# calderpg/voxelized_geometry_tools

Hardware: AMD Instinct MI355X
Metric: Mvoxels/s for 1024^3 float SDF extract @1 GPU; % HBM roofline (higher is better)
Workload: dtype int32; 1 GPU; 1024^3 float SDF, D1 spheres seed 42, res 0.01, device-resident; workload_key=c4, parallelism=single GPU, edt_variant=0

## Files before the change

### voxelized_geometry_tools_amd/csrc/edt_sweep_kernels.hip

```cpp
#include "edt_device.hpp"
#include "edt_line_geom.hpp"

#include <cstdlib>
#include <type_traits>

namespace vgt
{
namespace
{
#ifndef VGT_SWEEP_BAND
#define VGT_SWEEP_BAND 16
#endif
#ifndef VGT_SWEEP_RING
#define VGT_SWEEP_RING 32
#endif
#ifndef VGT_SWEEP_CHUNK
#define VGT_SWEEP_CHUNK 8
#endif
#ifndef VGT_SWEEP_WAVES
#define VGT_SWEEP_WAVES 4
#endif
#ifndef VGT_SWEEP_GROUP
#define VGT_SWEEP_GROUP 2
#endif
constexpr int kBand = VGT_SWEEP_BAND;
constexpr int kWord = 32;
#ifndef VGT_SWEEP_RING_WIDE
#define VGT_SWEEP_RING_WIDE 16
#endif
#ifndef VGT_SWEEP_CHUNK_WIDE
#define VGT_SWEEP_CHUNK_WIDE 4
#endif
#ifndef VGT_SWEEP_GROUPS
#define VGT_SWEEP_GROUPS 8
#endif
constexpr int kSweepGroups = VGT_SWEEP_GROUPS;
constexpr int kCounterStride = 32;
constexpr int kMaxSweepSlots = 4096;
template <bool kPacked>
struct RingShape
{
  static constexpr int kRing = kPacked ? VGT_SWEEP_RING : VGT_SWEEP_RING_WIDE;
  static constexpr int kChunk = kPacked ? VGT_SWEEP_CHUNK : VGT_SWEEP_CHUNK_WIDE;
  static_assert(kBand % kChunk == 0 && kRing >= 4 * kChunk && (kRing & (kRing - 1)) == 0 && kChunk % 4 == 0, "sizes");
};
constexpr int kFar = 32768;
static_assert(kWord % kBand == 0 && kBand % 2 == 0, "sizes");
#ifdef VGT_HOST_EMULATION
uint64_t class_band_tally[3] = {0, 0, 0};
#endif


template <bool kPacked>
struct Codec;
template <>
struct Codec<true>
{
  using Entry = uint32_t;
  static constexpr int32_t kSentinelG = (1 << 22) - 3;
  static __device__ __forceinline__ Entry Pack(int32_t G, int row)
  {
    return (static_cast<uint32_t>(G) << 10) | static_cast<uint32_t>(row);
  }
  static __device__ __forceinline__ int32_t G(Entry e) { return static_cast<int32_t>(e >> 10); }
  static __device__ __forceinline__ int Row(Entry e) { return static_cast<int>(e & 1023u); }
  static __device__ __forceinline__ Entry Unknown() { return ~0u; }
  static __device__ __forceinline__ bool IsUnknown(Entry e) { return e == ~0u; }
};
template <>
struct Codec<false>
{
  using Entry = uint2;
  static constexpr int32_t kSentinelG = 1 << 30;
  static __device__ __forceinline__ Entry Pack(int32_t G, int row)
  {
    return make_uint2(static_cast<uint32_t>(G), static_cast<uint32_t>(row));
  }
  static __device__ __forceinline__ int32_t G(Entry e) { return static_cast<int32_t>(e.x); }
  static __device__ __forceinline__ int Row(Entry e) { return static_cast<int>(e.y); }
  static __device__ __forceinline__ Entry Unknown() { return make_uint2(0u, ~0u); }
  static __device__ __forceinline__ bool IsUnknown(Entry e) { return e.y == ~0u; }
};

#ifndef VGT_SWEEP_NT
#define VGT_SWEEP_NT 3
#endif
__device__ __forceinline__ void StoreQuad(uint4* p, uint32_t a, uint32_t b, uint32_t c, uint32_t d)
{
#if defined(VGT_HOST_EMULATION) || !(VGT_SWEEP_NT & 8)
  *p = make_uint4(a, b, c, d);
#else
  using Raw = uint32_t __attribute__((ext_vector_type(4)));
  Raw r;
  r.x = a; r.y = b; r.z = c; r.w = d;
  __builtin_nontemporal_store(r, reinterpret_cast<Raw*>(p));
#endif
}
__device__ __forceinline__ uint4 LoadQuad(const uint4* p)
{
#if defined(VGT_HOST_EMULATION) || !(VGT_SWEEP_NT & 8)
  return *p;
#else
  using Raw = uint32_t __attribute__((ext_vector_type(4)));
  const Raw r = __builtin_nontemporal_load(reinterpret_cast<const Raw*>(p));
  return make_uint4(r.x, r.y, r.z, r.w);
#endif
}
__device__ __forceinline__ void StorePair(uint2* p, uint32_t a, uint32_t b)
{
#if defined(VGT_HOST_EMULATION) || !(VGT_SWEEP_NT & 4)
  *p = make_uint2(a, b);
#else
  using Raw = uint32_t __attribute__((ext_vector_type(2)));
  Raw r;
  r.x = a; r.y = b;
  __builtin_nontemporal_store(r, reinterpret_cast<Raw*>(p));
#endif
}
__device__ __forceinline__ uint2 LoadPair(const uint2* p)
{
#if defined(VGT_HOST_EMULATION) || !(VGT_SWEEP_NT & 4)
  return *p;
#else
  using Raw = uint32_t __attribute__((ext_vector_type(2)));
  const Raw r = __builtin_nontemporal_load(reinterpret_cast<const Raw*>(p));
  return make_uint2(r.x, r.y);
#endif
}

template <int N>
__device__ __forceinline__ void StoreChunk(uint32_t* dst, const uint32_t (&e)[N])
{
#pragma unroll
  for (int j = 0; j < N / 4; j++)
    StoreQuad(reinterpret_cast<uint4*>(dst) + j, e[4 * j], e[4 * j + 1], e[4 * j + 2], e[4 * j + 3]);
}
template <int N>
__device__ __forceinline__ void LoadChunk(const uint32_t* src, uint32_t (&e)[N])
{
#pragma unroll
  for (int j = 0; j < N / 4; j++)
  {
    const uint4 a = LoadQuad(reinterpret_cast<const uint4*>(src) + j);
    e[4 * j] = a.x;
    e[4 * j + 1] = a.y;
    e[4 * j + 2] = a.z;
    e[4 * j + 3] = a.w;
  }
}
template <int N>
__device__ __forceinline__ void StoreChunk(uint2* dst, const uint2 (&e)[N])
{
#pragma unroll
  for (int j = 0; j < N / 2; j++)
    StoreQuad(reinterpret_cast<uint4*>(dst) + j, e[2 * j].x, e[2 * j].y, e[2 * j + 1].x, e[2 * j + 1].y);
}
template <int N>
__device__ __forceinline__ void LoadChunk(const uint2* src, uint2 (&e)[N])
{
#pragma unroll
  for (int j = 0; j < N / 2; j++)
  {
    const uint4 a = LoadQuad(reinterpret_cast<const uint4*>(src) + j);
    e[2 * j] = make_uint2(a.x, a.y);
    e[2 * j + 1] = make_uint2(a.z, a.w);
  }
}

#ifdef VGT_HOST_EMULATION
#define VGT_GLOBAL
#else
#define VGT_GLOBAL __attribute__((address_space(1)))
#endif
template <typename T>
__device__ __forceinline__ VGT_GLOBAL T* UniformPointer(const VGT_GLOBAL T* p)
{
  const uint64_t v = reinterpret_cast<uint64_t>(p);
  const uint32_t lo = __builtin_amdgcn_readfirstlane(static_cast<uint32_t>(v));
  const uint32_t hi = __builtin_amdgcn_readfirstlane(static_cast<uint32_t>(v >> 32));
  return reinterpret_cast<VGT_GLOBAL T*>((static_cast<uint64_t>(hi) << 32) | lo);
}
template <typename T>
__device__ __forceinline__ VGT_GLOBAL T* GlobalPointer(T* p)
{
#ifdef VGT_HOST_EMULATION
  return p;
#else
  return reinterpret_cast<VGT_GLOBAL T*>(reinterpret_cast<uint64_t>(p));
#endif
}

__device__ __forceinline__ int32_t Mad24Uniform(int32_t a, int32_t b_uniform, int32_t c)
{
#ifdef VGT_HOST_EMULATION
  return a * b_uniform + c;
#else
  int32_t d;
  asm("v_mad_i32_i24 %0, %1, %2, %3" : "=v"(d) : "v"(a), "s"(b_uniform), "v"(c));
  return d;
#endif
}

__device__ __forceinline__ int32_t FreshCopy(int32_t v)
{
#ifdef VGT_HOST_EMULATION
  return v;
#else
  int32_t d;
  asm("v_mov_b32 %0, %1" : "=v"(d) : "v"(v));
  return d;
#endif
}

template <bool kInPlace>
__device__ __forceinline__ uint32_t PinnedOffset(uint32_t& byte_offset)
{
#ifndef VGT_HOST_EMULATION
  if constexpr (kInPlace)
    asm volatile("" : "+v"(byte_offset));
  else
  {
    uint32_t copy = byte_offset;
    asm volatile("" : "+v"(copy));
    return copy;
  }
#endif
  return byte_offset;
}
template <typename T>
__device__ __forceinline__ const VGT_GLOBAL T* LaneAddress(const VGT_GLOBAL T* row, uint32_t& byte_offset)
{
  return reinterpret_cast<const VGT_GLOBAL T*>(reinterpret_cast<const VGT_GLOBAL unsigned char*>(row) +
                                                PinnedOffset<false>(byte_offset));
}
template <typename T>
__device__ __forceinline__ VGT_GLOBAL T* LaneAddress(VGT_GLOBAL T* row, uint32_t& byte_offset)
{
  return reinterpret_cast<VGT_GLOBAL T*>(reinterpret_cast<VGT_GLOBAL unsigned char*>(row) +
                                         PinnedOffset<true>(byte_offset));
}

__device__ __forceinline__ uint32_t AbsDiffPlusOne(uint32_t a, uint32_t b_uniform)
{
  return (max(a, b_uniform) - min(a, b_uniform)) + 1u;
}
__device__ __forceinline__ uint32_t SpreadLaneMask(uint64_t mask_uniform, [[maybe_unused]] int lane)
{
#ifdef VGT_HOST_EMULATION
  return ((mask_uniform >> lane) & 1ull) ? ~0u : 0u;
#else
  return __builtin_amdgcn_inverse_ballot_w64(mask_uniform) ? ~0u : 0u;
#endif
}

__device__ __forceinline__ uint32_t LowBits(int bits)
{
  return (bits >= 32) ? ~0u : ((1u << bits) - 1u);
}

#if defined(VGT_HOST_EMULATION) || !(VGT_SWEEP_NT & 1)
#define VGT_STREAM_LOAD(p) (*(p))
#else
#define VGT_STREAM_LOAD(p) __builtin_nontemporal_load(p)
#endif
#if defined(VGT_HOST_EMULATION) || !(VGT_SWEEP_NT & 2)
#define VGT_STREAM_STORE(v, p) (*(p) = (v))
#else
#define VGT_STREAM_STORE(v, p) __builtin_nontemporal_store(v, p)
#endif

#ifdef VGT_HOST_EMULATION
#define VGT_COLD_PATH()
#define VGT_MIN_F32(acc, v) acc = fminf(acc, v)
#define VGT_MAX_F32(acc, v) acc = fmaxf(acc, v)
#define VGT_MIN3_F32(acc, a, b) acc = fminf(acc, fminf(a, b))
#define VGT_MAX3_F32(acc, a, b) acc = fmaxf(acc, fmaxf(a, b))
#else
#define VGT_COLD_PATH() asm volatile("; rare path")
#define VGT_MIN_F32(acc, v) asm("v_min_f32 %0, %0, %1" : "+v"(acc) : "v"(v))
#define VGT_MAX_F32(acc, v) asm("v_max_f32 %0, %0, %1" : "+v"(acc) : "v"(v))
#define VGT_MIN3_F32(acc, a, b) asm("v_min3_f32 %0, %0, %1, %2" : "+v"(acc) : "v"(a), "v"(b))
#define VGT_MAX3_F32(acc, a, b) asm("v_max3_f32 %0, %0, %1, %2" : "+v"(acc) : "v"(a), "v"(b))
#endif


__device__ __forceinline__ void WaveMinMax(float lo_value, float hi_value, uint32_t* minmax_enc)
{
  uint32_t lo = 0xffffffffu, hi = 0u;
  if (lo_value <= hi_value)
  {
    lo = EncodeOrdered(lo_value);
    hi = EncodeOrdered(hi_value);
  }
#ifdef VGT_HOST_EMULATION
  minmax_enc[0] = min(minmax_enc[0], lo);
  minmax_enc[1] = max(minmax_enc[1], hi);
#else
  for (int off = kWaveSize / 2; off > 0; off >>= 1)
  {
    lo = min(lo, static_cast<uint32_t>(__shfl_xor(static_cast<int>(lo), off)));
    hi = max(hi, static_cast<uint32_t>(__shfl_xor(static_cast<int>(hi), off)));
  }
  if (threadIdx.x == 0)
  {
    atomicMin(&minmax_enc[0], lo);
    atomicMax(&minmax_enc[1], hi);
  }
#endif
}

template <typename InT, typename OutT, bool kFinal, bool kPacked, bool kPlain>
__global__ __launch_bounds__(kWaveSize, VGT_SWEEP_WAVES) void SweepPassKernel(const InT* __restrict__ in,
                                                                            OutT* __restrict__ out,
                                                                            unsigned char* __restrict__ spill,
                                                                            uint2* __restrict__ word_info,
                                                                            uint32_t* __restrict__ minmax_enc,
                                                                            int* __restrict__ work_counter,
                                                                            const SweepGeom g)
{
  using C = Codec<kPacked>;
  using Entry = typename C::Entry;
  constexpr bool kRecords = std::is_same<InT, ClassRecord>::value;
  static_assert(!(kRecords && kFinal), "records feed the Y pass");
  constexpr int kRing = RingShape<kPacked>::kRing;
  constexpr int kChunk = RingShape<kPacked>::kChunk;
  constexpr int32_t kLimit = C::kSentinelG;
  constexpr int kEntryBytes = static_cast<int>(sizeof(Entry));
  constexpr int kShift = kPacked ? 8 : 9;
  constexpr uint32_t kSlot = 1u << kShift;
  constexpr uint32_t kRingMask = (kRing - 1) << kShift;
  constexpr int kChunkBytes = kChunk * kEntryBytes;
  constexpr uint32_t kChunkSlots = static_cast<uint32_t>(kChunk) << kShift;
  __shared__ Entry ring[kRing * kWaveSize];
  unsigned char* const ring_bytes = reinterpret_cast<unsigned char*>(ring);

  const int lane = threadIdx.x;
  const int n = g.n;
  const int64_t rstride = g.row_stride;
  unsigned char* const own_spill = spill + static_cast<int64_t>(blockIdx.x) * g.chunks * (kWaveSize * kChunkBytes);
  uint2* const own_info = word_info + static_cast<int64_t>(blockIdx.x) * (g.nwords + 1) * kWaveSize;
  const uint32_t lane_entry = static_cast<uint32_t>(lane) * kEntryBytes;
  const uint32_t lane_chunk = static_cast<uint32_t>(lane) * kChunkBytes;
  float lo_value = INFINITY, hi_value = -INFINITY;
  constexpr bool kUseTable = kFinal && kPlain && kPacked && (1024 / kBand <= 64);
  constexpr uint32_t kSmallD2 = 512;
  [[maybe_unused]] float* small_table = nullptr;
  if constexpr (kUseTable)
  {
    __shared__ float small_table_storage[kSmallD2];
    small_table = small_table_storage;
#ifdef VGT_HOST_EMULATION
    for (uint32_t d2 = 0; d2 < kSmallD2; d2++)
#else
    for (uint32_t d2 = static_cast<uint32_t>(lane); d2 < kSmallD2; d2 += kWaveSize)
#endif
      small_table[d2] = SqrtTimesResolutionExact(static_cast<int32_t>(d2), g.resolution);
    __syncthreads();
  }
#ifdef VGT_HOST_EMULATION
  int emulated_round = 0;
#endif
  [[maybe_unused]] auto fetch_item = [&]() -> int {
    int fetched = 0;
#ifndef VGT_HOST_EMULATION
    const int group = static_cast<int>(blockIdx.x) % g.groups;
    if (lane == 0) fetched = atomicAdd(work_counter + group * kCounterStride, 1);
    fetched = __builtin_amdgcn_readfirstlane(fetched);
    const int dealt = fetched / g.zsegs;
    fetched = (dealt * g.groups + group) * g.zsegs + (fetched - dealt * g.zsegs);
#endif
    return fetched;
  };
  for (;;)
  {
  int item = 0;
  unsigned char* wave_spill = own_spill;
  uint2* wave_info = own_info;
#ifdef VGT_HOST_EMULATION
  item = static_cast<int>(blockIdx.x + gridDim.x * emulated_round++);
#else
  item = fetch_item();
#endif
  if (item >= g.items) break;
  const int outer = item / g.zsegs;
  const int z0 = (item - outer * g.zsegs) * kWaveSize;
  const bool batched = g.batch_outers != g.outers;
  const int batch_index = batched ? outer / g.batch_outers : 0;
  const int outer_in_grid = outer - batch_index * g.batch_outers;
  const int64_t outer_offset = static_cast<int64_t>(outer) * g.outer_stride + static_cast<int64_t>(batch_index) * g.batch_skip;
  const uint32_t zl = static_cast<uint32_t>(min(lane, g.nz - 1 - z0));
  [[maybe_unused]] uint32_t lane_bytes = zl * 4u;
  const InT* const wave_in = kRecords ? in + static_cast<int64_t>(item) * n : in + (outer_offset + z0);
  OutT* const wave_out = out + (outer_offset + z0);

  uint32_t D = 4u << kShift, L = 0;
  int32_t Gt = C::kSentinelG, nB = 1;
  int rt = 0, A = 0;
  Entry e3 = C::Pack(C::kSentinelG + 2, 0);
  auto ring_ref = [&](uint32_t scaled_index) -> Entry& {
    return *reinterpret_cast<Entry*>(ring_bytes + ((scaled_index & kRingMask) | lane_entry));
  };
  auto chunk_in_ring = [&](uint32_t scaled_first) -> Entry* {
    return reinterpret_cast<Entry*>(ring_bytes + ((scaled_first & kRingMask) | lane_entry));
  };
  auto chunk_slot = [&](Entry* slots, uint32_t scaled_first, int j) -> Entry& {
    if constexpr (kPacked)
      return slots[j * kWaveSize];
    else
      return ring_ref(scaled_first + (static_cast<uint32_t>(j) << kShift));
  };
  static_assert(kRing % kChunk == 0, "a chunk must not wrap inside the ring");
  auto spill_ptr = [&](uint32_t scaled_first) -> Entry* {
    return reinterpret_cast<Entry*>(wave_spill + (scaled_first + lane_chunk));
  };
  ring_ref(0u << kShift) = C::Pack(0, 0);
  ring_ref(1u << kShift) = C::Pack(C::kSentinelG + 2, 0);
  ring_ref(2u << kShift) = C::Pack(C::kSentinelG + 1, 0);
  ring_ref(3u << kShift) = C::Pack(C::kSentinelG, 0);

  Entry pf0[kChunk], pf1[kChunk];
  int pf_count = 0;
  auto refill_now = [&]() {
    L -= kChunkSlots;
    const Entry* src = spill_ptr(L);
    Entry* const slots = chunk_in_ring(L);
#pragma unroll 1
    for (int j = 0; j < kChunk; j += 2)
    {
      const Entry a = src[j], b = src[j + 1];
      chunk_slot(slots, L, j) = a;
      chunk_slot(slots, L, j + 1) = b;
    }
    pf_count = 0;
  };
  auto pop = [&](auto third_in_register) {
    Gt += nB;
    rt -= A;
    if constexpr (decltype(third_in_register)::value)
    {
#ifdef VGT_HOST_EMULATION
      assert(!C::IsUnknown(e3));
#endif
    }
    else
    {
#ifdef VGT_HOST_EMULATION
      assert(C::IsUnknown(e3));
#endif
      if (__builtin_expect(D - 3 * kSlot < L, 0)) refill_now();
      e3 = ring_ref(D - 3 * kSlot);
    }
    A = rt - C::Row(e3);
    nB = C::G(e3) - Gt;
    D -= kSlot;
    e3 = C::Unknown();
  };
  auto commit = [&](const Entry (&buf)[kChunk]) {
    L -= kChunkSlots;
    Entry* const slots = chunk_in_ring(L);
#pragma unroll
    for (int j = 0; j < kChunk; j++) chunk_slot(slots, L, j) = buf[j];
  };

  uint32_t any_transition = 0;
  [[maybe_unused]] uint64_t small_bands = 0;
  {
    auto check_ring = [&]() {
      const uint32_t resident = D - L;
      const bool refilling = static_cast<int>(pf_count != 0) |
                             (static_cast<int>(L != 0) & static_cast<int>(resident <= kChunkSlots));
      if (__builtin_expect(__builtin_amdgcn_ballot_w64(refilling) != 0ull, 0))
      {
        VGT_COLD_PATH();
        if (pf_count != 0)
        {
          commit(pf0);
          pf_count = 0;
        }
        if (static_cast<int>(L != 0) & static_cast<int>(D - L <= kChunkSlots))
        {
          LoadChunk(spill_ptr(L - kChunkSlots), pf0);
          pf_count = 1;
        }
      }
      while (__builtin_amdgcn_ballot_w64(D - L > (static_cast<uint32_t>(kRing - kChunk) << kShift)) != 0ull)
      {
        if (D - L > (static_cast<uint32_t>(kRing - kChunk) << kShift))
        {
          Entry buf[kChunk];
          Entry* const slots = chunk_in_ring(L);
#pragma unroll
          for (int j = 0; j < kChunk; j++) buf[j] = chunk_slot(slots, L, j);
          StoreChunk(spill_ptr(L), buf);
          L += kChunkSlots;
        }
      }
    };

    int din = kFar;
    uint32_t prev_bit = 0;
    uint32_t sw = 0;
    const int32_t n2m = 2 * (n - 1);
    auto site = [&](int q, int32_t G, bool wanted) {
      int32_t dG = G - Gt;
      int dr = q - rt;
      if (static_cast<int>(wanted) & static_cast<int>(dG < static_cast<int32_t>(__umul24(n2m, dr))))
      {
        if (static_cast<int64_t>(dG) * A + static_cast<int64_t>(nB) * dr < 0)
        {
          pop(std::true_type{});
          dG = G - Gt;
          dr = q - rt;
          if (__builtin_expect(static_cast<int64_t>(dG) * A + static_cast<int64_t>(nB) * dr < 0, 0))
          {
            do
            {
              pop(std::false_type{});
              dG = G - Gt;
              dr = q - rt;
            } while (static_cast<int64_t>(dG) * A + static_cast<int64_t>(nB) * dr < 0);
          }
        }
        ring_ref(D) = C::Pack(G, q);
        e3 = C::Pack(Gt + nB, rt - A);
        A = dr;
        nB = -dG;
        Gt = G;
        rt = q;
        D += kSlot;
      }
#ifndef VGT_HOST_EMULATION
      asm volatile("" : "+v"(Gt));
#endif
    };
    auto band_done = [&](int r0, uint32_t bits) {
      const int sub = r0 & (kWord - 1);
      sw |= (bits >> (32 - kBand)) << sub;
      if (sub + kBand == kWord || r0 + kBand >= n)
      {
        const int word_first = r0 - sub;
        const int valid = min(kWord, n - word_first);
        uint32_t xdn = sw ^ ((sw << 1) | prev_bit);
        xdn &= LowBits(valid);
        if (word_first == 0) xdn &= ~1u;
        StorePair(wave_info + static_cast<int64_t>(word_first / kWord) * kWaveSize + lane, sw, static_cast<uint32_t>(din));
        any_transition |= xdn;
        din = xdn ? (valid - (31 - __clz(static_cast<int>(xdn)))) : min(din + valid, kFar);
        prev_bit = (sw >> (valid - 1)) & 1u;
        sw = 0;
      }
    };
    if constexpr (kRecords)
    {
      constexpr int kRows = 4;
      constexpr int kBlock = 64;
      static_assert(kBand % kRows == 0 && kChunk % kRows == 0 && kBlock % kBand == 0, "sizes");
      static_assert(3 * kBlock <= kRecordPadding, "reads past the end stay inside the padding");
      const uint32_t xq = 2u * zl + (kRecordBias - 1u);
      [[maybe_unused]] auto load_block = [&](int first_row) -> uint4 {
#ifdef VGT_HOST_EMULATION
        return make_uint4(0u, 0u, 0u, 0u);
#else
        using Raw = uint32_t __attribute__((ext_vector_type(4)));
        const Raw r = *(reinterpret_cast<const Raw*>(wave_in + first_row) + lane);
        return make_uint4(r.x, r.y, r.z, r.w);
#endif
      };
      auto block_marks = [&]([[maybe_unused]] const uint4& blk, [[maybe_unused]] int first_row, uint64_t& marks,
                             uint64_t& filled) {
#ifdef VGT_HOST_EMULATION
        marks = filled = 0;
        for (int l = 0; l < kBlock; l++)
        {
          const ClassRecord r = wave_in[first_row + l];
          if (r.above2 == kRecordNoSite) marks |= 1ull << l;
          if (r.mask_lo & 1u) filled |= 1ull << l;
        }
#else
        marks = __builtin_amdgcn_ballot_w64(blk.w == kRecordNoSite);
        filled = __builtin_amdgcn_ballot_w64((blk.x & 1u) != 0u);
#endif
      };
      auto record_of = [&]([[maybe_unused]] const uint4& blk, [[maybe_unused]] int first_row, int index) -> uint4 {
#ifdef VGT_HOST_EMULATION
        const ClassRecord r = wave_in[first_row + index];
        return make_uint4(r.mask_lo, r.mask_hi, r.below2, r.above2);
#else
        return make_uint4(__builtin_amdgcn_readlane(blk.x, index), __builtin_amdgcn_readlane(blk.y, index),
                          __builtin_amdgcn_readlane(blk.z, index), __builtin_amdgcn_readlane(blk.w, index));
#endif
      };
      auto row = [&](int q, const uint4& rec, uint32_t& bits) {
        const uint64_t m = (static_cast<uint64_t>(rec.y) << 32) | rec.x;
        bits = __builtin_amdgcn_alignbit(SpreadLaneMask(m, lane), bits, 1);
        uint32_t f2 = min(AbsDiffPlusOne(xq, rec.z), AbsDiffPlusOne(xq, rec.w));
        if (__builtin_expect(static_cast<int64_t>(m) != (static_cast<int64_t>(m) >> 63), 0))
        {
          uint64_t own = (m ^ (m >> 1)) & 0x7fffffffffffffffull;
          const uint32_t t1 = 2u * static_cast<uint32_t>(__ffsll(static_cast<long long>(own)) - 1) + kRecordBias;
          own &= own - 1ull;
          uint32_t t2 = t1;
          if (own)
          {
            t2 = 2u * static_cast<uint32_t>(__ffsll(static_cast<long long>(own)) - 1) + kRecordBias;
            own &= own - 1ull;
          }
          f2 = min(f2, min(AbsDiffPlusOne(xq, t1), AbsDiffPlusOne(xq, t2)));
          if (__builtin_expect(own != 0ull, 0))
          {
            VGT_COLD_PATH();
            do
            {
              const uint32_t t = 2u * static_cast<uint32_t>(__ffsll(static_cast<long long>(own)) - 1) + kRecordBias;
              f2 = min(f2, AbsDiffPlusOne(xq, t));
              own &= own - 1ull;
            } while (own != 0ull);
          }
        }
        const int32_t f = static_cast<int32_t>(f2 >> 1);
        site(q, __mul24(f, f) + q * q, f2 < 2u * static_cast<uint32_t>(kInf16));
      };
      uint4 blk0 = load_block(0), blk1 = load_block(kBlock), blk2 = load_block(2 * kBlock);
      uint64_t marks = 0, filled = 0;
      constexpr uint32_t kBandMask = kBand >= 32 ? ~0u : ((1u << (kBand % 32)) - 1u);
      for (int r0 = 0; r0 < n; r0 += kBand)
      {
        __builtin_assume(r0 >= 0 && r0 < 16384);
        const int in_block = r0 & (kBlock - 1);
        const int block_first = r0 - in_block;
        if (in_block == 0)
        {
          if (r0 != 0)
          {
            blk0 = blk1;
            blk1 = blk2;
            blk2 = load_block(r0 + 2 * kBlock);
          }
          block_marks(blk0, r0, marks, filled);
        }
        const uint32_t band_marks = static_cast<uint32_t>(marks >> in_block) & kBandMask;
        const uint32_t band_filled = static_cast<uint32_t>(filled >> in_block) & kBandMask;
        uint32_t bits;
        if (band_marks == kBandMask && r0 + kBand <= n)
        {
          bits = band_filled << (32 - kBand);
        }
        else
        {
          bits = 0;
#pragma unroll
          for (int k0 = 0; k0 < kBand; k0 += kRows)
          {
            const int q0 = r0 + k0;
            if (k0 % kChunk == 0) check_ring();
            if (((band_marks >> k0) & 0xfu) == 0xfu && q0 + kRows <= n)
              bits = __builtin_amdgcn_alignbit((band_filled >> k0) & 0xfu, bits, kRows);
            else
            {
#pragma unroll
              for (int k = 0; k < kRows; k++)
              {
                if (q0 + k < n)
                  row(q0 + k, record_of(blk0, block_first, in_block + k0 + k), bits);
                else
                  bits >>= 1;
              }
            }
          }
        }
        band_done(r0, bits);
      }
    }
    else
    {
      static_assert(kRecords || kFinal, "the X pass reads the Y pass's field");
      auto load_band = [&](int32_t (&dst)[kBand], int first_row) {
        const VGT_GLOBAL InT* row_in = UniformPointer(GlobalPointer(wave_in + static_cast<int64_t>(first_row) * rstride));
        if (first_row + kBand <= n)
        {
  #pragma unroll
          for (int k = 0; k < kBand; k++)
          {
            dst[k] = static_cast<int32_t>(VGT_STREAM_LOAD(LaneAddress(row_in, lane_bytes)));
            row_in = UniformPointer(row_in + rstride);
          }
        }
        else
        {
  #pragma unroll
          for (int k = 0; k < kBand; k++)
          {
            dst[k] = static_cast<int32_t>(VGT_STREAM_LOAD(LaneAddress(row_in, lane_bytes)));
            if (first_row + k + 1 < n) row_in = UniformPointer(row_in + rstride);
          }
        }
      };
      int32_t nxt[kBand];
      load_band(nxt, 0);
      constexpr int32_t kNoSiteG = 0x60000000;
      auto decode = [&](int32_t v, int q, int32_t& G) {
        const int32_t f = static_cast<int32_t>(min(static_cast<uint32_t>(v) & 0x7fffffffu, static_cast<uint32_t>(kNoSiteG)));
        G = f + q * q;
      };
      int32_t G_prev = kNoSiteG, G_cur = 0;
      decode(nxt[0], 0, G_cur);
      for (int r0 = 0; r0 < n; r0 += kBand)
      {
        __builtin_assume(r0 >= 0 && r0 < 16384);
        int32_t cur[kBand];
#pragma unroll
        for (int k = 0; k < kBand; k++) cur[k] = nxt[k];
        if (r0 + kBand < n) load_band(nxt, r0 + kBand);
        if constexpr (kUseTable)
        {
          uint32_t any = 0u;
#pragma unroll
          for (int k = 0; k < kBand; k++) any |= static_cast<uint32_t>(cur[k]);
          if (r0 + kBand <= n && __builtin_amdgcn_ballot_w64((any & 0x7fffffffu) >= kSmallD2) == 0ull)
            small_bands |= 1ull << (r0 / kBand);
        }
        uint32_t bits = 0;
        auto rows = [&](auto guarded) {
          constexpr bool kGuard = decltype(guarded)::value;
#pragma unroll
          for (int k = 0; k < kBand; k++)
          {
            if (k % kChunk == 0) check_ring();
            if (kGuard && r0 + k >= n) bits <<= 1;
            if (!kGuard || r0 + k < n)
            {
              const int q = r0 + k;
              bits = __builtin_amdgcn_alignbit(bits, static_cast<uint32_t>(cur[k]), 31);
              int32_t G_next = kNoSiteG + (q + 1) * (q + 1);
              if ((!kGuard && k + 1 < kBand) || q + 1 < n) decode(k + 1 < kBand ? cur[k + 1] : nxt[0], q + 1, G_next);
              site(q, G_cur, G_cur - G_prev < G_next - G_cur);
              G_prev = G_cur;
              G_cur = G_next;
            }
          }
        };
        if (r0 + kBand <= n)
          rows(std::false_type{});
        else
          rows(std::true_type{});
        band_done(r0, __builtin_bitreverse32(bits));
      }
    }
  }

  const bool classes = __builtin_amdgcn_ballot_w64(any_transition != 0u) != 0ull;
  const bool any_empty = __builtin_amdgcn_ballot_w64(D == (4u << kShift)) != 0ull;
  bool all_empty = !classes && __builtin_amdgcn_ballot_w64(D != (4u << kShift)) == 0ull;
  if constexpr (kFinal && !kPlain) all_empty = all_empty && !g.add_virtual_border;
  if (all_empty)
  {
    const int nwords = g.nwords;
    VGT_GLOBAL OutT* row_out = UniformPointer(GlobalPointer(wave_out + static_cast<int64_t>(n - 1) * rstride));
    uint2 info = LoadPair(wave_info + static_cast<int64_t>(nwords - 1) * kWaveSize + lane);
    for (int w = nwords - 1; w >= 0; w--)
    {
      const uint32_t sw = info.x;
      if (w > 0) info = LoadPair(wave_info + static_cast<int64_t>(w - 1) * kWaveSize + lane);
      const int valid = min(kWord, n - w * kWord);
      if constexpr (kFinal)
      {
        const uint32_t rows_mask = LowBits(valid);
        if (sw & rows_mask) lo_value = -INFINITY;
        if (~sw & rows_mask) hi_value = INFINITY;
      }
      for (int k = valid - 1; k >= 0; k--)
      {
        const uint32_t sign = (sw >> k) << 31;
        if constexpr (kFinal)
        {
          VGT_STREAM_STORE(__uint_as_float(0x7f800000u | sign), LaneAddress(row_out, lane_bytes));
        }
        else
        {
          VGT_STREAM_STORE(static_cast<OutT>(static_cast<uint32_t>(kInf32) | sign), LaneAddress(row_out, lane_bytes));
        }
        row_out = UniformPointer(row_out - rstride);
      }
    }
  }
  else
  {
    pf_count = 0;
    auto refill_step = [&]() {
      const bool refilling =
          static_cast<int>(pf_count != 0) |
          (static_cast<int>(L != 0) & static_cast<int>(D - L <= (static_cast<uint32_t>(kRing - kChunk) << kShift)));
      if (__builtin_amdgcn_ballot_w64(refilling) != 0ull)
      {
        if (pf_count > 0) commit(pf0);
        if (pf_count > 1) commit(pf1);
        pf_count = 0;
        const uint32_t resident = D - L;
        if (static_cast<int>(L != 0) & static_cast<int>(resident <= (static_cast<uint32_t>(kRing - kChunk) << kShift)))
        {
          LoadChunk(spill_ptr(L - kChunkSlots), pf0);
          pf_count = 1;
          if (static_cast<int>(L != kChunkSlots) &
              static_cast<int>(resident <= (static_cast<uint32_t>(kRing - 2 * kChunk) << kShift)))
          {
            LoadChunk(spill_ptr(L - 2 * kChunkSlots), pf1);
            pf_count = 2;
          }
        }
      }
    };
    constexpr int kStep = (kChunk < 8) ? 8 : kChunk;

    if (C::IsUnknown(e3))
    {
      if (D - 3 * kSlot < L) refill_now();
      e3 = ring_ref(D - 3 * kSlot);
    }
    int A2 = (rt - A) - C::Row(e3);
    int32_t nB2 = C::G(e3) - (Gt + nB);
    if (__builtin_expect(D - 4 * kSlot < L, 0)) refill_now();
    Entry e4 = ring_ref(D - 4 * kSlot);
    auto pop_down = [&]() {
      Gt += nB;
      rt -= A;
      A = FreshCopy(A2);
      nB = FreshCopy(nB2);
      A2 = (rt - A) - C::Row(e4);
      nB2 = C::G(e4) - (Gt + nB);
      D -= kSlot;
      if (__builtin_expect(D - 4 * kSlot < L, 0)) refill_now();
      e4 = ring_ref(D - 4 * kSlot);
    };

    int dn = kFar;
    uint32_t above_bit0 = 0;
    const int nwords = g.nwords;
    uint2 info = LoadPair(wave_info + static_cast<int64_t>(nwords - 1) * kWaveSize + lane);
    uint2 info_below = make_uint2(0u, 0u);
    if (nwords > 1) info_below = LoadPair(wave_info + static_cast<int64_t>(nwords - 2) * kWaveSize + lane);
    uint2 info_next = make_uint2(0u, 0u);
    uint32_t xdn_word = 0, xup_word = 0;
    VGT_GLOBAL OutT* row_out = UniformPointer(GlobalPointer(wave_out + static_cast<int64_t>(n - 1) * rstride));
    const int last_band = (n - 1) / kBand * kBand;
    for (int r0 = last_band; r0 >= 0; r0 -= kBand)
    {
      __builtin_assume(r0 >= 0 && r0 < 16384);
      const int sub = r0 & (kWord - 1);
      if (sub + kBand == kWord || r0 == last_band)
      {
        const int w = r0 / kWord;
        if (r0 != last_band)
        {
          above_bit0 = info.x & 1u;
          info = info_below;
          info_below = info_next;
        }
        if (w > 1) info_next = LoadPair(wave_info + static_cast<int64_t>(w - 2) * kWaveSize + lane);
        if (classes)
        {
          const uint32_t sw = info.x;
          const int valid = min(kWord, n - w * kWord);
          const uint32_t prev_bit = (w > 0) ? (info_below.x >> (kWord - 1)) : (sw & 1u);
          xdn_word = sw ^ ((sw << 1) | prev_bit);
          xup_word = sw ^ ((sw >> 1) | (above_bit0 << (kWord - 1)));
          if (r0 == last_band) xup_word &= ~(1u << (valid - 1));
        }
      }
      const uint32_t swb = info.x >> sub;
      int dp[8];
      uint32_t xup = 0;
      if (classes) xup = xup_word >> sub;
      auto rows = [&](auto guarded, auto with_classes, auto from_table) {
        constexpr bool kGuard = decltype(guarded)::value;
        constexpr bool kClasses = decltype(with_classes)::value;
        constexpr bool kTable = decltype(from_table)::value;
        constexpr int kGroup = kGuard ? 1 : VGT_SWEEP_GROUP;
        [[maybe_unused]] float& lo_acc = lo_value;
        [[maybe_unused]] float& hi_acc = hi_value;
        [[maybe_unused]] uint32_t grp_best[kGroup];
        [[maybe_unused]] int32_t grp_sign[kGroup];
#pragma unroll
        for (int k = kBand - 1; k >= 0; k--)
        {
          if (k % kStep == kStep - 1) refill_step();
          if (kClasses && k % 8 == 7)
          {
            const int first = sub + k - 7;
            const uint32_t below = xdn_word & LowBits(first);
            int d = below ? (first - (31 - __clz(static_cast<int>(below)))) : static_cast<int>(info.y) + first;
            const uint32_t xdn = xdn_word >> first;
#pragma unroll
            for (int j = 0; j < 8; j++)
            {
              d = ((xdn >> j) & 1u) ? 1 : d + 1;
              dp[j] = d;
            }
          }
          if (!kGuard || r0 + k < n)
          {
            const int q = r0 + k;
            const int q2 = 2 * q;
            __builtin_assume(A >= 0 && A < 16384 && A2 >= 0 && A2 < 16384 && rt >= 0 && rt < 16384);
            int32_t t1 = Mad24Uniform(A, q2, nB);
            int32_t t2 = Mad24Uniform(A2, q2, nB2);
            if (__builtin_expect(__builtin_amdgcn_ballot_w64(t2 <= 0) != 0ull, 0))
            {
              do
              {
                if (t1 <= 0)
                {
                  pop_down();
                  __builtin_assume(A2 >= 0 && A2 < 16384);
                  t1 = t2;
                  t2 = Mad24Uniform(A2, q2, nB2);
                }
              } while (__builtin_amdgcn_ballot_w64(t2 <= 0) != 0ull);
              __builtin_assume(rt >= 0 && rt < 16384);
            }
            uint32_t best = static_cast<uint32_t>(Mad24Uniform(rt, -q2, Gt) + q * q + min(t1, 0));
            if constexpr (kClasses)
            {
              dn = ((xup >> k) & 1u) ? 1 : dn + 1;
              const uint32_t dm = static_cast<uint32_t>(min(dp[k & 7], dn));
              best = min(best, dm * dm);
            }
            const int32_t sign = __builtin_amdgcn_sbfe(static_cast<int32_t>(swb), k, 1);
            if constexpr (kFinal)
            {
              grp_best[k % kGroup] = best;
              grp_sign[k % kGroup] = sign;
              if (k % kGroup == 0)
              {
                float dist[kGroup];
                uint32_t d2s[kGroup];
                bool redo[kGroup], none[kGroup];
                bool any_rare = false;
                if constexpr (kTable)
                {
#pragma unroll
                  for (int j = kGroup - 1; j >= 0; j--)
                  {
#ifdef VGT_HOST_EMULATION
                    assert(grp_best[j] < kSmallD2);
#endif
                    dist[j] = small_table[grp_best[j]];
                    redo[j] = none[j] = false;
                    d2s[j] = 0;
                  }
                }
                else
                {
#pragma unroll
                for (int j = kGroup - 1; j >= 0; j--)
                {
                  uint32_t d2 = grp_best[j];
                  bool exact = false;
                  if constexpr (!kPlain)
                  {
                    if (g.add_virtual_border)
                    {
                      const int qq = q + j;
                      const int x = (g.pass_axis == 0) ? qq : outer_in_grid + g.outer_begin;
                      const int y = (g.pass_axis == 0) ? outer_in_grid + g.outer_begin : qq;
                      const int32_t site = (d2 >= static_cast<uint32_t>(kLimit)) ? kInf32 : static_cast<int32_t>(d2);
                      const int32_t clamped = ClampToVirtualBorder(site, x, y, z0 + static_cast<int>(zl) + g.z_offset, g.nx,
                                                                   g.ny, g.nz_global);
                      d2 = (clamped == kInf32) ? static_cast<uint32_t>(kLimit) : static_cast<uint32_t>(clamped);
                    }
                    exact = !(g.resolution > 1.0e-30 && g.resolution < 1.0e30);
                  }
                  bool unsure;
                  dist[j] = FastSqrtTimesResolution(d2, g.resolution, unsure);
                  none[j] = kClasses && d2 >= static_cast<uint32_t>(kLimit);
                  redo[j] = unsure || exact;
                  d2s[j] = d2;
                  any_rare = any_rare || redo[j] || none[j];
                }
                }
                if (!kTable && __builtin_expect(__builtin_amdgcn_ballot_w64(any_rare) != 0ull, 0))
                {
                  VGT_COLD_PATH();
#pragma unroll
                  for (int j = 0; j < kGroup; j++)
                  {
                    if (redo[j]) dist[j] = SqrtTimesResolutionExact(static_cast<int32_t>(d2s[j]), g.resolution);
                    if (none[j]) dist[j] = __uint_as_float(0x7f800000u);
                  }
                }
                float value[kGroup];
                VGT_GLOBAL OutT* store_at = row_out;
#pragma unroll
                for (int j = kGroup - 1; j >= 0; j--)
                {
                  value[j] = __uint_as_float(__float_as_uint(dist[j]) | (static_cast<uint32_t>(grp_sign[j]) & 0x80000000u));
                  VGT_STREAM_STORE(value[j], LaneAddress(store_at, lane_bytes));
                  store_at = UniformPointer(store_at - rstride);
                }
                row_out = store_at;
#pragma unroll
                for (int j = kGroup - 1; j >= 0; j -= 2)
                {
                  if (j >= 1)
                  {
                    VGT_MIN3_F32(lo_acc, value[j], value[j - 1]);
                    VGT_MAX3_F32(hi_acc, value[j], value[j - 1]);
                  }
                  else
                  {
                    VGT_MIN_F32(lo_acc, value[j]);
                    VGT_MAX_F32(hi_acc, value[j]);
                  }
                }
              }
            }
            else
            {
              const int32_t d2 =
                  (kClasses && best >= static_cast<uint32_t>(kLimit)) ? kInf32 : static_cast<int32_t>(best);
              VGT_STREAM_STORE(static_cast<OutT>(d2 | (sign & static_cast<int32_t>(0x80000000u))), LaneAddress(row_out, lane_bytes));
              row_out = UniformPointer(row_out - rstride);
            }
          }
        }
      };
      bool small_band = false;
      if constexpr (kUseTable) small_band = ((small_bands >> (r0 / kBand)) & 1ull) != 0ull;
      bool without_candidates = false;
      if (classes && !any_empty && r0 + kBand <= n)
      {
        constexpr uint32_t kBandMask = kBand >= 32 ? ~0u : ((1u << (kBand % 32)) - 1u);
        const uint32_t touched = ((xdn_word | xup_word) >> sub) & kBandMask;
#ifdef VGT_HOST_EMULATION
        int ran = 2;
#endif
        if (__builtin_amdgcn_ballot_w64(touched != 0u) == 0ull)
        {
          const uint32_t below = xdn_word & LowBits(sub);
          const int d = below ? (sub - (31 - __clz(static_cast<int>(below)))) : static_cast<int>(info.y) + sub;
          const uint32_t delta = static_cast<uint32_t>(min(d, dn) + 1);
          __builtin_assume(rt >= 0 && rt < 16384);
          const int qt = r0 + kBand - 1;
          const int32_t p_first = Mad24Uniform(rt, -2 * r0, Gt) + r0 * r0;
          const int32_t p_last = Mad24Uniform(rt, -2 * qt, Gt) + qt * qt;
          const uint32_t B = static_cast<uint32_t>(max(p_first, p_last));
          const bool needed = static_cast<int>(B >= static_cast<uint32_t>(kLimit)) | static_cast<int>(B > delta * delta);
          without_candidates = __builtin_amdgcn_ballot_w64(needed) == 0ull;
          if (without_candidates) dn += kBand;
#ifdef VGT_HOST_EMULATION
          ran = without_candidates ? 1 : 0;
#endif
        }
#ifdef VGT_HOST_EMULATION
        if (any_transition != 0u) class_band_tally[ran]++;
#endif
      }
      const bool class_rows = classes && !without_candidates;
      if (r0 + kBand > n)
        rows(std::true_type{}, std::true_type{}, std::false_type{});
      else if (small_band)
      {
        if constexpr (kUseTable)
        {
          if (class_rows)
            rows(std::false_type{}, std::true_type{}, std::true_type{});
          else
            rows(std::false_type{}, std::false_type{}, std::true_type{});
        }
      }
      else if (class_rows || any_empty)
        rows(std::false_type{}, std::true_type{}, std::false_type{});
      else
        rows(std::false_type{}, std::false_type{}, std::false_type{});
      if (classes) dn = min(dn, kFar);
    }
  }
  if constexpr (kFinal)
  {
    if (batched)
    {
      WaveMinMax(lo_value, hi_value, minmax_enc + 2 * batch_index);
      lo_value = INFINITY;
      hi_value = -INFINITY;
    }
  }
  }
  if constexpr (kFinal) WaveMinMax(lo_value, hi_value, minmax_enc);
}

#ifdef VGT_HOST_EMULATION
constexpr int64_t kSweepSlots = 3;
#else
constexpr int64_t kSweepSlots = kMaxSweepSlots;
#endif
constexpr size_t kCounterBytes = (kSweepGroups * kCounterStride * sizeof(int) + 255) / 256 * 256;

int64_t SpillChunks(int64_t n, int chunk) { return (n + 4 + chunk - 1) / chunk + 1; }

bool PackedEntries(int64_t n, int64_t max_input)
{
  return n <= 1024 && max_input + (n - 1) * (n - 1) < Codec<true>::kSentinelG;
}

size_t SlotScratchBytes(int64_t n, bool packed)
{
  const int64_t nwords = (n + kWord - 1) / kWord;
  const size_t spill = packed ? SpillChunks(n, RingShape<true>::kChunk) * kWaveSize * RingShape<true>::kChunk * sizeof(uint32_t)
                              : SpillChunks(n, RingShape<false>::kChunk) * kWaveSize * RingShape<false>::kChunk * sizeof(uint2);
  return spill + static_cast<size_t>(nwords + 1) * kWaveSize * sizeof(uint2);
}

size_t PassScratchBytes(int64_t n, int64_t items, int64_t max_input)
{
  const int64_t slots = items < kSweepSlots ? items : kSweepSlots;
  const size_t planned = static_cast<size_t>(slots) * SlotScratchBytes(n, PackedEntries(n, max_input));
  const size_t one_wide = SlotScratchBytes(n, false);
  return kCounterBytes + (planned > one_wide ? planned : one_wide);
}

template <typename InT, typename OutT, bool kFinal>
hipError_t LaunchSweep(const InT* in, OutT* out, void* scratch, size_t scratch_bytes, uint32_t* minmax_enc, SweepGeom g,
                       int64_t outer_count, int64_t max_input, hipStream_t stream)
{
  g.zsegs = (g.nz + kWaveSize - 1) / kWaveSize;
  g.nwords = (g.n + kWord - 1) / kWord;
  const int64_t items = outer_count * g.zsegs;
  if (items <= 0) return hipSuccess;
  if (items > 0x7fffffffLL) return hipErrorInvalidValue;
  g.items = static_cast<int>(items);
  g.outers = static_cast<int>(outer_count);
  if (g.batch_outers <= 0)
  {
    g.batch_outers = g.outers;
    g.batch_skip = 0;
  }
  const bool packed = PackedEntries(g.n, max_input);
  int64_t slots = items < kSweepSlots ? items : kSweepSlots;
  {
    const size_t per_slot = SlotScratchBytes(g.n, packed);
    const int64_t fit = scratch_bytes > kCounterBytes ? static_cast<int64_t>((scratch_bytes - kCounterBytes) / per_slot) : 0;
    if (fit < 1) return hipErrorInvalidValue;
    if (fit < slots) slots = fit;
  }
  g.groups = static_cast<int>(slots < kSweepGroups ? slots : kSweepGroups);
  const int chunk = packed ? RingShape<true>::kChunk : RingShape<false>::kChunk;
  g.chunks = static_cast<int>(SpillChunks(g.n, chunk));
  char* bytes = static_cast<char*>(scratch);
  int* counter = reinterpret_cast<int*>(bytes);
  unsigned char* spill = reinterpret_cast<unsigned char*>(bytes + kCounterBytes);
  const size_t spill_bytes =
      static_cast<size_t>(slots) * g.chunks * kWaveSize * chunk * (packed ? sizeof(uint32_t) : sizeof(uint2));
  uint2* info = reinterpret_cast<uint2*>(bytes + kCounterBytes + spill_bytes);
#ifdef VGT_HOST_EMULATION
  *counter = 0;
#endif
  const dim3 grid(static_cast<unsigned>(slots)), block(kWaveSize);
  const bool general = kFinal && (g.add_virtual_border || !(g.resolution > 1.0e-30 && g.resolution < 1.0e30));
#ifndef VGT_HOST_EMULATION
  {
    const hipError_t err = hipMemsetAsync(counter, 0, kSweepGroups * kCounterStride * sizeof(int), stream);
    if (err != hipSuccess) return err;
  }
#endif
#define VGT_LAUNCH_SWEEP(PACKED, PLAIN)                                                                             \
  hipLaunchKernelGGL((SweepPassKernel<InT, OutT, kFinal, PACKED, PLAIN>), grid, block, 0, stream, in, out, spill, info, \
                     minmax_enc, counter, g)
  if (packed && general)
    VGT_LAUNCH_SWEEP(true, !kFinal);
  else if (packed)
    VGT_LAUNCH_SWEEP(true, true);
  else if (general)
    VGT_LAUNCH_SWEEP(false, !kFinal);
  else
    VGT_LAUNCH_SWEEP(false, true);
#undef VGT_LAUNCH_SWEEP
  return hipGetLastError();
}


int64_t MaxInputY(const SdfParams& p)
{
  const int64_t nzg = p.nz_global > 0 ? p.nz_global : p.nz;
  return (nzg - 1) * (nzg - 1);
}
int64_t MaxInputX(const SdfParams& p) { return MaxInputY(p) + (p.ny - 1) * (p.ny - 1); }
}

size_t SweepPassScratchBytes(int64_t nx, int64_t ny, int64_t nz, int64_t batch)
{
  const int64_t zsegs = (nz + kWaveSize - 1) / kWaveSize;
  const int64_t max_y = (nz - 1) * (nz - 1), max_x = max_y + (ny - 1) * (ny - 1);
  const size_t y = PassScratchBytes(ny, batch * nx * zsegs, max_y), x = PassScratchBytes(nx, batch * ny * zsegs, max_x);
  return (y > x ? y : x) + 256;
}

hipError_t LaunchPassYSweepRecords(const ClassRecord* records, int32_t* out32, SweepScratch scratch, const SdfParams& p,
                                   hipStream_t stream)
{
#ifndef VGT_HOST_EMULATION
  if (p.ny <= ShortLineLimit(p.nx * ((p.nz + kWaveSize - 1) / kWaveSize))) return LaunchPassYShortRecords(records, out32, p, stream);
#endif
  int64_t outer_count = 0;
  const SweepGeom g = SweepGeometry(p, 1, &outer_count);
  return LaunchSweep<ClassRecord, int32_t, false>(records, out32, scratch.ptr, scratch.bytes, nullptr, g, outer_count,
                                                  MaxInputY(p), stream);
}

hipError_t LaunchPassXSweepFinalizeRange(const int32_t* in32, float* sdf, uint32_t* minmax_enc, SweepScratch scratch,
                                         const SdfParams& p, int64_t outer_begin, int64_t outer_count_or_all,
                                         hipStream_t stream)
{
  int64_t outer_count = 0;
  SweepGeom g = SweepGeometry(p, 0, &outer_count);
  if (p.batch > 1)
  {
    if (outer_count_or_all >= 0 || p.batch * outer_count > 0x7fffffffLL) return hipErrorInvalidValue;
    g.batch_outers = static_cast<int>(outer_count);
    g.batch_skip = (p.nx - 1) * p.ny * p.nz;
    outer_count *= p.batch;
  }
  if (outer_count_or_all >= 0)
  {
    in32 += outer_begin * g.outer_stride;
    sdf += outer_begin * g.outer_stride;
    g.outer_begin = static_cast<int>(outer_begin);
    outer_count = outer_count_or_all;
  }
  return LaunchSweep<int32_t, float, true>(in32, sdf, scratch.ptr, scratch.bytes, minmax_enc, g, outer_count,
                                           MaxInputX(p), stream);
}

hipError_t LaunchPassXSweepFinalize(const int32_t* in32, float* sdf, uint32_t* minmax_enc, SweepScratch scratch,
                                    const SdfParams& p, hipStream_t stream)
{
  return LaunchPassXSweepFinalizeRange(in32, sdf, minmax_enc, scratch, p, 0, -1, stream);
}

}
```

Baseline: 238,300 Mvoxels/s.

## Reschedule block and sign-word prefetches and drop wave-uniform spill loop

```diff
diff --git a/voxelized_geometry_tools_amd/csrc/edt_sweep_kernels.hip b/voxelized_geometry_tools_amd/csrc/edt_sweep_kernels.hip
--- a/voxelized_geometry_tools_amd/csrc/edt_sweep_kernels.hip
+++ b/voxelized_geometry_tools_amd/csrc/edt_sweep_kernels.hip
@@ -48,6 +48,7 @@
 static_assert(kWord % kBand == 0 && kBand % 2 == 0, "sizes");
 #ifdef VGT_HOST_EMULATION
 uint64_t class_band_tally[3] = {0, 0, 0};
+uint64_t ring_checks = 0, ring_spills = 0;
 #endif
 
 
@@ -251,6 +252,20 @@
 #else
   return __builtin_amdgcn_inverse_ballot_w64(mask_uniform) ? ~0u : 0u;
 #endif
+}
+
+__device__ __forceinline__ void TakeLoaded([[maybe_unused]] uint32_t& v)
+{
+#ifndef VGT_HOST_EMULATION
+  asm volatile("" : "+v"(v));
+#endif
+}
+__device__ __forceinline__ void TakeLoaded(uint4& v)
+{
+  TakeLoaded(v.x);
+  TakeLoaded(v.y);
+  TakeLoaded(v.z);
+  TakeLoaded(v.w);
 }
 
 __device__ __forceinline__ uint32_t LowBits(int bits)
@@ -321,6 +336,7 @@
   using C = Codec<kPacked>;
   using Entry = typename C::Entry;
   constexpr bool kRecords = std::is_same<InT, ClassRecord>::value;
+  constexpr bool kTakeSignWords = kFinal;
   static_assert(!(kRecords && kFinal), "records feed the Y pass");
   constexpr int kRing = RingShape<kPacked>::kRing;
   constexpr int kChunk = RingShape<kPacked>::kChunk;
@@ -483,18 +499,22 @@
           pf_count = 1;
         }
       }
-      while (__builtin_amdgcn_ballot_w64(D - L > (static_cast<uint32_t>(kRing - kChunk) << kShift)) != 0ull)
+      if (D - L > (static_cast<uint32_t>(kRing - kChunk) << kShift))
       {
-        if (D - L > (static_cast<uint32_t>(kRing - kChunk) << kShift))
-        {
-          Entry buf[kChunk];
-          Entry* const slots = chunk_in_ring(L);
-#pragma unroll
-          for (int j = 0; j < kChunk; j++) buf[j] = chunk_slot(slots, L, j);
-          StoreChunk(spill_ptr(L), buf);
-          L += kChunkSlots;
-        }
+        Entry buf[kChunk];
+        Entry* const slots = chunk_in_ring(L);
+#pragma unroll
+        for (int j = 0; j < kChunk; j++) buf[j] = chunk_slot(slots, L, j);
+        StoreChunk(spill_ptr(L), buf);
+        L += kChunkSlots;
+#ifdef VGT_HOST_EMULATION
+        ring_spills++;
+#endif
       }
+#ifdef VGT_HOST_EMULATION
+      ring_checks++;
+      assert(D - L <= (static_cast<uint32_t>(kRing - kChunk) << kShift));
+#endif
     };
 
     int din = kFar;
@@ -621,6 +641,7 @@
         site(q, __mul24(f, f) + q * q, f2 < 2u * static_cast<uint32_t>(kInf16));
       };
       uint4 blk0 = load_block(0), blk1 = load_block(kBlock), blk2 = load_block(2 * kBlock);
+      TakeLoaded(blk0);
       uint64_t marks = 0, filled = 0;
       constexpr uint32_t kBandMask = kBand >= 32 ? ~0u : ((1u << (kBand % 32)) - 1u);
       for (int r0 = 0; r0 < n; r0 += kBand)
@@ -628,16 +649,7 @@
         __builtin_assume(r0 >= 0 && r0 < 16384);
         const int in_block = r0 & (kBlock - 1);
         const int block_first = r0 - in_block;
-        if (in_block == 0)
-        {
-          if (r0 != 0)
-          {
-            blk0 = blk1;
-            blk1 = blk2;
-            blk2 = load_block(r0 + 2 * kBlock);
-          }
-          block_marks(blk0, r0, marks, filled);
-        }
+        if (in_block == 0) block_marks(blk0, r0, marks, filled);
         const uint32_t band_marks = static_cast<uint32_t>(marks >> in_block) & kBandMask;
         const uint32_t band_filled = static_cast<uint32_t>(filled >> in_block) & kBandMask;
         uint32_t bits;
@@ -668,6 +680,19 @@
             }
           }
         }
+        int moves_up = static_cast<int>(in_block + kBand == kBlock && r0 + kBand < n);
+        if (moves_up)
+        {
+          blk0 = blk1;
+          blk1 = blk2;
+          TakeLoaded(blk0);
+          TakeLoaded(blk1);
+        }
+#ifndef VGT_HOST_EMULATION
+        asm volatile("" : "+v"(moves_up));
+        moves_up = __builtin_amdgcn_readfirstlane(moves_up);
+#endif
+        if (moves_up) blk2 = load_block(r0 + kBand + 2 * kBlock);
         band_done(r0, bits);
       }
     }
@@ -839,6 +864,13 @@
     uint2 info_below = make_uint2(0u, 0u);
     if (nwords > 1) info_below = LoadPair(wave_info + static_cast<int64_t>(nwords - 2) * kWaveSize + lane);
     uint2 info_next = make_uint2(0u, 0u);
+    if constexpr (kTakeSignWords)
+    {
+      TakeLoaded(info.x);
+      TakeLoaded(info.y);
+      TakeLoaded(info_below.x);
+      TakeLoaded(info_below.y);
+    }
     uint32_t xdn_word = 0, xup_word = 0;
     VGT_GLOBAL OutT* row_out = UniformPointer(GlobalPointer(wave_out + static_cast<int64_t>(n - 1) * rstride));
     const int last_band = (n - 1) / kBand * kBand;
@@ -855,7 +887,6 @@
           info = info_below;
           info_below = info_next;
         }
-        if (w > 1) info_next = LoadPair(wave_info + static_cast<int64_t>(w - 2) * kWaveSize + lane);
         if (classes)
         {
           const uint32_t sw = info.x;
@@ -866,6 +897,12 @@
           if (r0 == last_band) xup_word &= ~(1u << (valid - 1));
         }
       }
+      const bool word_begins = sub + kBand == kWord || r0 == last_band;
+      [[maybe_unused]] uint2 info_fresh = make_uint2(0u, 0u);
+      if constexpr (kTakeSignWords)
+        info_fresh = LoadPair(wave_info + static_cast<int64_t>(max(r0 / kWord - 2, 0)) * kWaveSize + lane);
+      else if (word_begins && r0 >= 2 * kWord)
+        info_next = LoadPair(wave_info + static_cast<int64_t>(r0 / kWord - 2) * kWaveSize + lane);
       const uint32_t swb = info.x >> sub;
       int dp[8];
       uint32_t xup = 0;
@@ -1022,6 +1059,12 @@
             }
           }
         }
+        if constexpr (kTakeSignWords)
+        {
+          TakeLoaded(info_fresh.x);
+          TakeLoaded(info_fresh.y);
+          if (word_begins) info_next = info_fresh;
+        }
       };
       bool small_band = false;
       if constexpr (kUseTable) small_band = ((small_bands >> (r0 / kBand)) & 1ull) != 0ull;
```

Measured after the change: 245,300 Mvoxels/s (median of 6 runs). 1.03x the previous value.
